# HITSZ-NRSL/De6D

Hardware: AMD Instinct MI355X
Metric: scenes/sec (16384-pt KITTI) at 1/2/4/8 MI355X; 3D mAP parity vs ref (higher is better)
Workload: dtype f32

## Files before the change

### de6d_amd/csrc/mlp_group.hip

```cpp
#include "common.h"
#include "compact_list.h"
#include "mfma_tile.h"

namespace {

D6_GEMM_PRIO_DECL


struct GroupArgs {
  int rows;
  const float *p; int ldp; int pcol0;
  const float *w1; int ldw1; const float *s1;
  const float *w2; int ldw2; const float *s2;
  const float *w3; int ldw3; const float *s3;
  const float *pts; int ldpts;
  const float *ctr; int ldctr;
  const int *idx; int n, m, ns; const int *cnt;
  const int *hdr; const int *crow_p; const int *crow_c;
  float *y; int ldy; int col0;
  int pre;
  int yvec;
  int *ticket;
};

__device__ __forceinline__ int g_draw_ticket(int *ticket, int grid) {
  return grid + __hip_atomic_fetch_add(ticket, 1, __ATOMIC_RELAXED, __HIP_MEMORY_SCOPE_AGENT);
}
__device__ __forceinline__ void g_leave(int *ticket, int workers) {
  const int gone = __hip_atomic_fetch_add(ticket + 1, 1, __ATOMIC_RELAXED, __HIP_MEMORY_SCOPE_AGENT);
  if (gone == workers - 1) {
    __hip_atomic_store(ticket, 0, __ATOMIC_RELAXED, __HIP_MEMORY_SCOPE_AGENT);
    __hip_atomic_store(ticket + 1, 0, __ATOMIC_RELAXED, __HIP_MEMORY_SCOPE_AGENT);
  }
}

template <int TN> constexpr int kGroupVW = TN >= 4 ? 4 : TN;
template <int TN>
__device__ __forceinline__ int tile_col(int j, int l31) {
  constexpr int VW = kGroupVW<TN>;
  return (j / VW) * (32 * VW) + VW * l31 + (j % VW);
}

template <int VW> struct BVec;
template <> struct BVec<1> { typedef float T; };
template <> struct BVec<2> { typedef f32x2 T; };
template <> struct BVec<4> { typedef f32x4 T; };

template <int VW>
__device__ __forceinline__ void g_store_group(float *rowptr, const float (&v)[VW], const int tag, float *__restrict__ scr,
                                              const int lane, const int yvec) {
  const bool live = tag >= 0;
  const int l31 = lane & 31;
  if constexpr (VW == 1) {
    if (live) d6_compact_store(rowptr + l31, v[0], tag);
  } else {
    if (!yvec) {
#pragma unroll
      for (int t = 0; t < VW; ++t)
        if (live) d6_compact_store(rowptr + VW * l31 + t, v[t], tag);
      return;
    }
    const bool atomic = live && (tag & kCompactTagSplit);
    typename BVec<VW>::T pack;
#pragma unroll
    for (int t = 0; t < VW; ++t) pack[t] = v[t];
    if (live && !atomic) *reinterpret_cast<typename BVec<VW>::T *>(rowptr + VW * l31) = pack;
    if (__ballot(atomic) != 0ull) {
      *reinterpret_cast<typename BVec<VW>::T *>(scr + lane * VW) = pack;
      d6_lds_wave_sync();
      const float *half = scr + (lane & 32) * VW;
      float x[VW];
#pragma unroll
      for (int t = 0; t < VW; ++t) x[t] = half[32 * t + l31];
      d6_lds_wave_sync();
      if (atomic) {
#pragma unroll
        for (int t = 0; t < VW; ++t)
          __hip_atomic_fetch_max(reinterpret_cast<int *>(rowptr + 32 * t + l31), __builtin_bit_cast(int, x[t]), __ATOMIC_RELAXED,
                                 __HIP_MEMORY_SCOPE_AGENT);
      }
    }
  }
}

template <int VW>
__device__ __forceinline__ typename BVec<VW>::T load_b(const __amdgpu_buffer_rsrc_t srd, uint32_t voff, int soff) {
  if constexpr (VW == 4) return __builtin_bit_cast(typename BVec<4>::T, __builtin_amdgcn_raw_buffer_load_b128(srd, voff, soff, 0));
  else if constexpr (VW == 2) return __builtin_bit_cast(typename BVec<2>::T, __builtin_amdgcn_raw_buffer_load_b64(srd, voff, soff, 0));
  else return __builtin_bit_cast(float, __builtin_amdgcn_raw_buffer_load_b32(srd, voff, soff, 0));
}
template <int VW>
__device__ __forceinline__ float bget(const typename BVec<VW>::T &v, int i) {
  if constexpr (VW == 1) return v;
  else return v[i];
}

#ifdef DET6D_EXPERIMENTS
__device__ int d6_group_kmul = 1;
#define D6_KOFF(x) (d6_group_kmul * (x))
__device__ int d6_group_phase_c2 = 512, d6_group_phase_c3 = 1024;
__device__ unsigned long long d6_group_phase[8 + 18];
#define D6_PHASE_DECL const unsigned long long ph_c0 = clock64(); unsigned long long ph_w3 = 0, ph_w2 = 0, ph_wt = 0; unsigned long long ph_t = wall_clock64(), ph_acc[5] = {0, 0, 0, 0, 0}, ph_tiles = 0; const unsigned long long ph_start = ph_t; const bool ph_on = C3 == d6_group_phase_c3 && C2 == d6_group_phase_c2;
#define D6_PHASE(i) do { if (ph_on) { __builtin_amdgcn_sched_barrier(0); const unsigned long long now_ = wall_clock64(); ph_acc[i] += now_ - ph_t; ph_t = now_; __builtin_amdgcn_sched_barrier(0); } } while (0)
#define D6_WAVE_T0 do { if (ph_on) { __builtin_amdgcn_sched_barrier(0); ph_wt = wall_clock64(); __builtin_amdgcn_sched_barrier(0); } } while (0)
#define D6_WAVE_T1(x) do { if (ph_on) { __builtin_amdgcn_sched_barrier(0); x += wall_clock64() - ph_wt; __builtin_amdgcn_sched_barrier(0); } } while (0)
#define D6_PHASE_END do { if (ph_on && tid == 0) { for (int i_ = 0; i_ < 5; ++i_) atomicAdd(&d6_group_phase[i_], ph_acc[i_]); atomicAdd(&d6_group_phase[5], ph_tiles); atomicAdd(&d6_group_phase[6], wall_clock64() - ph_start); atomicAdd(&d6_group_phase[7], 1ull); atomicAdd(&d6_group_phase[8], clock64() - ph_c0); } if (ph_on && (tid & 63) == 0) { atomicAdd(&d6_group_phase[9 + (tid >> 6)], ph_w3); atomicAdd(&d6_group_phase[17 + (tid >> 6)], ph_w2); } } while (0)
#else
#define D6_PHASE_DECL
#define D6_PHASE(i)
#define D6_WAVE_T0
#define D6_WAVE_T1(x)
#define D6_PHASE_END
#define D6_KOFF(x) (x)
#endif

template <int K, int TN, int LDX>
struct GroupLayer {
  static constexpr int VW = kGroupVW<TN>;
  static constexpr int NV = TN / VW;
  static constexpr int KS = K / 2;
  static constexpr int UK = 32 / TN;
  static constexpr int NB = KS / UK;
  static_assert(KS % UK == 0 && NB >= 2, "block structure");
  typedef typename BVec<VW>::T bvec;
  bvec b0[UK][NV], b1[UK][NV], b2[UK][NV];

  __device__ __forceinline__ static void fetch(bvec (&b)[UK][NV], const __amdgpu_buffer_rsrc_t srd, const uint32_t voff,
                                               const int ldw_bytes, const int blk) {
#pragma unroll
    for (int u = 0; u < UK; ++u)
#pragma unroll
      for (int v = 0; v < NV; ++v) b[u][v] = load_b<VW>(srd, voff, D6_KOFF(2 * (blk * UK + u) * ldw_bytes) + 128 * VW * v);
  }
  __device__ __forceinline__ static void compute(const bvec (&b)[UK][NV], const float *__restrict__ X, f32x16 (&acc)[TN],
                                                 const int l31, const int kh, const int blk) {
    float a[UK];
    const float *xa = X + l31 * LDX + 2 * blk * UK + kh;
#pragma unroll
    for (int u = 0; u < UK; ++u) a[u] = xa[2 * u];
#pragma unroll
    for (int u = 0; u < UK; ++u)
#pragma unroll
      for (int j = 0; j < TN; ++j) d6_mfma(a[u], bget<VW>(b[u][j / VW], j % VW), acc[j]);
  }
  __device__ __forceinline__ void start(const __amdgpu_buffer_rsrc_t srd, const uint32_t voff, const int ldw_bytes) {
    fetch(b0, srd, voff, ldw_bytes, 0);
    fetch(b1, srd, voff, ldw_bytes, 1);
  }
  __device__ __forceinline__ void run(const float *__restrict__ X, const __amdgpu_buffer_rsrc_t srd, const uint32_t voff,
                                      const int ldw_bytes, f32x16 (&acc)[TN], const int l31, const int kh) {
    auto clamp = [](int blk) { return blk < NB ? blk : NB - 1; };
    int blk = 0;
#pragma unroll 1
    for (; blk + 3 <= NB; blk += 3) {
      fetch(b2, srd, voff, ldw_bytes, blk + 2);
      compute(b0, X, acc, l31, kh, blk);
      fetch(b0, srd, voff, ldw_bytes, clamp(blk + 3));
      compute(b1, X, acc, l31, kh, blk + 1);
      fetch(b1, srd, voff, ldw_bytes, clamp(blk + 4));
      compute(b2, X, acc, l31, kh, blk + 2);
    }
    if (blk < NB) {
      compute(b0, X, acc, l31, kh, blk);
      if (blk + 1 < NB) compute(b1, X, acc, l31, kh, blk + 1);
    }
  }
};

template <bool COMPACT, int EPR>
__device__ __forceinline__ void group_row_entry(const GroupArgs &g, const int tile, const int tid, int &e0, int &e1) {
  const int r = tile * 32 + tid / EPR;
  if (COMPACT) { e0 = g.crow_c[r]; e1 = g.crow_p[r]; }
  else { e0 = g.idx[r]; e1 = 0; }
}

template <int C1, bool COMPACT, int EPR>
__device__ __forceinline__ void group_layer1(const GroupArgs &g, const int tile, const int tid, float *__restrict__ X1,
                                             int *__restrict__ tagbuf, const int e0, const int e1) {
  constexpr int LD1 = C1 + 1;
  const int erow = tid / EPR, eq = tid % EPR;
    {
      const int r = tile * 32 + erow;
      long long prow;
      int cj;
      bool real = true;
      if (COMPACT) {
        const int tag = e0;
        if (eq == 0) tagbuf[erow] = tag;
        real = tag >= 0;
        cj = d6_compact_centre(tag);
        prow = e1;
      } else {
        cj = r / g.ns;
        prow = (long long)(cj / g.m) * g.n + e0;
      }
      float dx = 0.f, dy = 0.f, dz = 0.f;
      if (real) {
        const float *pt = g.pts + prow * g.ldpts;
        const float *ce = g.ctr + (long long)cj * g.ldctr;
        dx = pt[0] - ce[0]; dy = pt[1] - ce[1]; dz = pt[2] - ce[2];
      }
      const float *prow_p = g.p + (real ? prow : 0) * g.ldp + g.pcol0;
      float *xr = X1 + erow * LD1;
#pragma unroll 4
      for (int c = 4 * eq; c < C1; c += 4 * EPR) {
        const f32x4 pv = *reinterpret_cast<const f32x4 *>(prow_p + c);
        const f32x4 wx = *reinterpret_cast<const f32x4 *>(g.w1 + c);
        const f32x4 wy = *reinterpret_cast<const f32x4 *>(g.w1 + g.ldw1 + c);
        const f32x4 wz = *reinterpret_cast<const f32x4 *>(g.w1 + 2 * g.ldw1 + c);
        const f32x4 sh = *reinterpret_cast<const f32x4 *>(g.s1 + c);
#pragma unroll
        for (int e = 0; e < 4; ++e) {
          const float v = d6_relu(D6_FMA(dz, wz[e], D6_FMA(dy, wy[e], D6_FMA(dx, wx[e], pv[e]))) + sh[e]);
          xr[c + e] = real ? v : 0.f;
        }
      }
    }
}

template <int TN3, bool COMPACT>
__device__ __forceinline__ void group_pool_store(const GroupArgs &g, const int tile, f32x16 (&acc)[TN3], const float (&sh3)[TN3],
                                                 const int colbase, const int l31, const int kh, const int h1, const int h2,
                                                 const int h3, const int h4, const int h5, const int *__restrict__ tagbuf,
                                                 float *__restrict__ scr) {
    constexpr int VW = kGroupVW<TN3>;
    constexpr int NG = TN3 / VW;
    const int lane = l31 + 32 * kh;
    if (COMPACT) {
      const int sc = d6_compact_class(tile * 32, h1, h2, h3, h4, h5);
      if (sc < 4) {
#pragma unroll
        for (int e = 0; e < 16; ++e) {
          if (sc == 2 && (e & 1)) continue;
          const int tag = tagbuf[d6_acc_row(e) + 4 * kh];
          float *dst = g.y + (size_t)(tag < 0 ? 0 : tag & kCompactTagCentre) * g.ldy + g.col0 + colbase;
#pragma unroll
          for (int jg = 0; jg < NG; ++jg) {
            float v[VW];
#pragma unroll
            for (int t = 0; t < VW; ++t) {
              const int j = jg * VW + t;
              const float raw = sc == 2 ? d6_vmax(acc[j][e], acc[j][e + 1 < 16 ? e + 1 : e]) : acc[j][e];
              v[t] = d6_compact_is_empty(tag) ? 0.f : d6_relu(raw + sh3[j]);
            }
            g_store_group<VW>(dst + jg * 32 * VW, v, tag, scr, lane, g.yvec);
          }
        }
      } else {
        int oc[4];
#pragma unroll
        for (int qq = 0; qq < 4; ++qq) {
          const int rr = d6_compact_out_row(sc, qq, kh);
          oc[qq] = rr >= 0 ? tagbuf[rr] : -1;
        }
#pragma unroll
        for (int jg = 0; jg < NG; ++jg) {
          float q[VW][4];
#pragma unroll
          for (int t = 0; t < VW; ++t) {
            const int j = jg * VW + t;
#pragma unroll
            for (int qq = 0; qq < 4; ++qq)
              q[t][qq] = d6_acc_max4(acc[j], qq);
            d6_compact_pool(q[t], sc);
          }
#pragma unroll
          for (int qq = 0; qq < 4; ++qq) {
            float v[VW];
#pragma unroll
            for (int t = 0; t < VW; ++t) v[t] = d6_compact_is_empty(oc[qq]) ? 0.f : d6_relu(q[t][qq] + sh3[jg * VW + t]);
            float *dst = g.y + (size_t)(oc[qq] < 0 ? 0 : oc[qq] & kCompactTagCentre) * g.ldy + g.col0 + colbase + jg * 32 * VW;
            g_store_group<VW>(dst, v, oc[qq], scr, lane, g.yvec);
          }
        }
      }
    } else {
      const int c0 = g.ns == 32 ? tile : 2 * tile;
      const int cnt0 = g.cnt[c0], cnt1 = g.ns == 32 ? 0 : g.cnt[c0 + 1];
      const int plain = kh == 0 ? 0 : -1;
#pragma unroll
      for (int jg = 0; jg < NG; ++jg) {
        float v0[VW], v1[VW];
#pragma unroll
        for (int t = 0; t < VW; ++t) {
          const int j = jg * VW + t;
          float q[4];
#pragma unroll
          for (int qq = 0; qq < 4; ++qq) q[qq] = d6_half_max(d6_acc_max4(acc[j], qq));
          if (g.ns == 32) {
            const float mx = d6_relu(d6_vmax(d6_vmax(q[0], q[1]), d6_vmax(q[2], q[3])) + sh3[j]);
            v0[t] = cnt0 > 0 ? mx : 0.f;
            v1[t] = 0.f;
          } else {
            v0[t] = cnt0 > 0 ? d6_relu(d6_vmax(q[0], q[1]) + sh3[j]) : 0.f;
            v1[t] = cnt1 > 0 ? d6_relu(d6_vmax(q[2], q[3]) + sh3[j]) : 0.f;
          }
        }
        float *dst = g.y + g.col0 + colbase + jg * 32 * VW;
        g_store_group<VW>(dst + (size_t)c0 * g.ldy, v0, plain, scr, lane, g.yvec);
        if (g.ns != 32) g_store_group<VW>(dst + (size_t)(c0 + 1) * g.ldy, v1, plain, scr, lane, g.yvec);
      }
    }
}

template <int C1, int C2, int C3, bool COMPACT, int NW>
__global__ __launch_bounds__(64 * NW, (NW == 4 && C3 <= 256) ? 3 : 1) void mlp_group_kernel(const GroupArgs g) {
  D6_GEMM_PRIO_APPLY();
  constexpr int LD1 = C1 + 1, LD2 = C2 + 1;
  constexpr int TN2 = C2 / (32 * NW), TN3 = C3 / (32 * NW);
  static_assert(TN2 >= 1 && TN3 >= 1, "every wave needs at least one 32-column tile per layer");
  extern __shared__ float lds[];
  float *X1 = lds;
  float *X2 = lds + 32 * LD1;
  int *tags = reinterpret_cast<int *>(lds + 32 * (LD1 + LD2));
  int it = 0;
  const int tid = threadIdx.x, lane = tid & 63, wave = tid >> 6, l31 = lane & 31, kh = lane >> 5;
  float *scr = reinterpret_cast<float *>(tags + 64) + wave * (64 * kGroupVW<TN3>);
  const int live_tiles = (COMPACT ? g.hdr[kCompactHdrLive] : g.rows) / 32;
  if ((int)blockIdx.x >= live_tiles) return;
  int h1 = 0, h2 = 0, h3 = 0, h4 = 0, h5 = 0;
  if (COMPACT) d6_compact_class_ends(g.hdr, h1, h2, h3, h4, h5);

  const __amdgpu_buffer_rsrc_t srd2 = d6_buffer(g.w2);
  const __amdgpu_buffer_rsrc_t srd3 = d6_buffer(g.w3);
  const uint32_t voff2 = (uint32_t)(kh * g.ldw2 + wave * (C2 / NW) + tile_col<TN2>(0, l31)) * 4u;
  const uint32_t voff3 = (uint32_t)(kh * g.ldw3 + wave * (C3 / NW) + tile_col<TN3>(0, l31)) * 4u;
  float sh2[TN2], sh3[TN3];
#pragma unroll
  for (int j = 0; j < TN2; ++j) sh2[j] = g.s2[wave * (C2 / NW) + tile_col<TN2>(j, l31)];
#pragma unroll
  for (int j = 0; j < TN3; ++j) sh3[j] = g.s3[wave * (C3 / NW) + tile_col<TN3>(j, l31)];

  D6_PHASE_DECL
  int e0, e1;
  group_row_entry<COMPACT, 2 * NW>(g, blockIdx.x, tid, e0, e1);
  __shared__ int next_tile_s[2];
  int *const ticket = COMPACT ? g.ticket : nullptr;
  for (int tile = blockIdx.x; tile < live_tiles;) {
#ifdef DET6D_EXPERIMENTS
    ++ph_tiles;
#endif
    int drawn = 0;
    if (ticket && tid == 0) drawn = g_draw_ticket(ticket, (int)gridDim.x);
    GroupLayer<C1, TN2, LD1> second;
    GroupLayer<C2, TN3, LD2> third;
    second.start(srd2, voff2, g.ldw2 * 4);
    const int par = it & 1;
    int *tagbuf = tags + 32 * (it++ & 1);
    if (!g.pre) group_row_entry<COMPACT, 2 * NW>(g, tile, tid, e0, e1);
    group_layer1<C1, COMPACT, 2 * NW>(g, tile, tid, X1, tagbuf, e0, e1);
    if (ticket && tid == 0) next_tile_s[par] = drawn;
    __syncthreads();
    const int next_tile = ticket ? next_tile_s[par] : tile + (int)gridDim.x;
    D6_PHASE(0);
    {
      f32x16 acc[TN2];
#pragma unroll
      for (int j = 0; j < TN2; ++j) d6_acc_zero(acc[j]);
      D6_WAVE_T0;
      second.run(X1, srd2, voff2, g.ldw2 * 4, acc, l31, kh);
      third.start(srd3, voff3, g.ldw3 * 4);
      D6_WAVE_T1(ph_w2);
      D6_PHASE(1);
#pragma unroll
      for (int j = 0; j < TN2; ++j) {
        float *xc = X2 + wave * (C2 / NW) + tile_col<TN2>(j, l31);
#pragma unroll
        for (int e = 0; e < 16; ++e) xc[(d6_acc_row(e) + 4 * kh) * LD2] = d6_relu(acc[j][e] + sh2[j]);
      }
    }
    __syncthreads();
    D6_PHASE(2);
    f32x16 acc[TN3];
#pragma unroll
    for (int j = 0; j < TN3; ++j) d6_acc_zero(acc[j]);
    D6_WAVE_T0;
    if (g.pre) {
      const int nt = next_tile;
      group_row_entry<COMPACT, 2 * NW>(g, nt < live_tiles ? nt : tile, tid, e0, e1);
    }
    third.run(X2, srd3, voff3, g.ldw3 * 4, acc, l31, kh);
    D6_WAVE_T1(ph_w3);
    D6_PHASE(3);
    group_pool_store<TN3, COMPACT>(g, tile, acc, sh3, wave * (C3 / NW), l31, kh, h1, h2, h3, h4, h5, tagbuf, scr);
    D6_PHASE(4);
    tile = next_tile;
  }
  if (ticket && tid == 0) g_leave(ticket, min((int)gridDim.x, live_tiles));
  D6_PHASE_END;
}


template <int K, int TN, int LDX, int UK, int DEPTH>
__device__ __forceinline__ void stream_layer(const float *__restrict__ X, const __amdgpu_buffer_rsrc_t srd, const uint32_t voff,
                                             const int ldw_bytes, const int soff0, f32x16 (&acc)[TN], const int l31, const int kh) {
  constexpr int VW = kGroupVW<TN>;
  constexpr int NV = TN / VW;
  constexpr int KS = K / 2;
  constexpr int NB = KS / UK;
  static_assert(KS % UK == 0 && NB % DEPTH == 0 && NB >= DEPTH, "ring structure");
  typedef typename BVec<VW>::T bvec;
  bvec b[DEPTH][UK][NV];
  auto fetch = [&](bvec (&bs)[UK][NV], int blk) {
#pragma unroll
    for (int u = 0; u < UK; ++u)
#pragma unroll
      for (int v = 0; v < NV; ++v) bs[u][v] = load_b<VW>(srd, voff, soff0 + D6_KOFF(2 * (blk * UK + u) * ldw_bytes) + 128 * VW * v);
  };
  const float *xa = X + l31 * LDX + kh;
  float a[UK];
#pragma unroll
  for (int d = 0; d < DEPTH - 1; ++d) fetch(b[d], d);
#pragma unroll
  for (int u = 0; u < UK; ++u) a[u] = xa[2 * u];
#pragma unroll 1
  for (int blk = 0; blk < NB; blk += DEPTH) {
#pragma unroll
    for (int d = 0; d < DEPTH; ++d) {
      const int cur = blk + d;
      fetch(b[(d + DEPTH - 1) % DEPTH], cur + DEPTH - 1 < NB ? cur + DEPTH - 1 : NB - 1);
      float an[UK];
      const int nxt = cur + 1 < NB ? cur + 1 : cur;
#pragma unroll
      for (int u = 0; u < UK; ++u) an[u] = xa[2 * (nxt * UK + u)];
#pragma unroll
      for (int u = 0; u < UK; ++u)
#pragma unroll
        for (int j = 0; j < TN; ++j) d6_mfma(a[u], bget<VW>(b[d][u][j / VW], j % VW), acc[j]);
#pragma unroll
      for (int u = 0; u < UK; ++u) a[u] = an[u];
    }
  }
}

template <int C1, int C2, int C3, bool COMPACT>
__global__ __launch_bounds__(256, 2) void mlp_group_stream_kernel(const GroupArgs g) {
  D6_GEMM_PRIO_APPLY();
  constexpr int CH = 128;
  constexpr int NCH = C2 / CH;
  constexpr int LD1 = C1 + 1, LDY = CH + 1;
  constexpr int TN3 = C3 / 128;
  static_assert(C2 % CH == 0 && NCH >= 2 && TN3 >= 2, "chunk structure");
  extern __shared__ float lds[];
  float *X1 = lds;
  float *Y0 = lds + 32 * LD1;
  float *Y1 = Y0 + 32 * LDY;
  int *tags = reinterpret_cast<int *>(Y1 + 32 * LDY);
  int it = 0;
  const int tid = threadIdx.x, lane = tid & 63, wave = tid >> 6, l31 = lane & 31, kh = lane >> 5;
  float *scr = reinterpret_cast<float *>(tags + 64) + wave * (64 * kGroupVW<TN3>);
  const int live_tiles = (COMPACT ? g.hdr[kCompactHdrLive] : g.rows) / 32;
  if ((int)blockIdx.x >= live_tiles) return;
  int h1 = 0, h2 = 0, h3 = 0, h4 = 0, h5 = 0;
  if (COMPACT) d6_compact_class_ends(g.hdr, h1, h2, h3, h4, h5);

  const __amdgpu_buffer_rsrc_t srd2 = d6_buffer(g.w2);
  const __amdgpu_buffer_rsrc_t srd3 = d6_buffer(g.w3);
  const uint32_t voff2 = (uint32_t)(kh * g.ldw2 + 32 * wave + l31) * 4u;
  const uint32_t voff3 = (uint32_t)(kh * g.ldw3 + wave * (C3 / 4) + tile_col<TN3>(0, l31)) * 4u;
  float sh3[TN3];
#pragma unroll
  for (int j = 0; j < TN3; ++j) sh3[j] = g.s3[wave * (C3 / 4) + tile_col<TN3>(j, l31)];

  auto second = [&](const int c, float *__restrict__ Y) {
    const float sh2 = g.s2[CH * c + 32 * wave + l31];
    f32x16 acc2[1];
    d6_acc_zero(acc2[0]);
    stream_layer<C1, 1, LD1, 8, 4>(X1, srd2, voff2, g.ldw2 * 4, CH * c * 4, acc2, l31, kh);
    float *yc = Y + 32 * wave + l31;
#pragma unroll
    for (int e = 0; e < 16; ++e) yc[(d6_acc_row(e) + 4 * kh) * LDY] = d6_relu(acc2[0][e] + sh2);
  };

  __shared__ int next_tile_s[2];
  int *const ticket = COMPACT ? g.ticket : nullptr;
  for (int tile = blockIdx.x; tile < live_tiles;) {
    int drawn = 0;
    if (ticket && tid == 0) drawn = g_draw_ticket(ticket, (int)gridDim.x);
    const int par = it & 1;
    int *tagbuf = tags + 32 * (it++ & 1);
    int e0, e1;
    group_row_entry<COMPACT, 8>(g, tile, tid, e0, e1);
    group_layer1<C1, COMPACT, 8>(g, tile, tid, X1, tagbuf, e0, e1);
    if (ticket && tid == 0) next_tile_s[par] = drawn;
    __syncthreads();
    const int next_tile = ticket ? next_tile_s[par] : tile + (int)gridDim.x;
    f32x16 acc[TN3];
#pragma unroll
    for (int j = 0; j < TN3; ++j) d6_acc_zero(acc[j]);
    second(0, Y0);
    __syncthreads();
#pragma unroll 1
    for (int c = 0; c < NCH; ++c) {
      float *Yc = (c & 1) ? Y1 : Y0;
      float *Yn = (c & 1) ? Y0 : Y1;
      stream_layer<CH, TN3, LDY, 16 / TN3 >= 1 ? 16 / TN3 : 1, 4>(Yc, srd3, voff3, g.ldw3 * 4, CH * c * g.ldw3 * 4, acc, l31, kh);
      if (c + 1 < NCH) {
        second(c + 1, Yn);
        __syncthreads();
      }
    }
    group_pool_store<TN3, COMPACT>(g, tile, acc, sh3, wave * (C3 / 4), l31, kh, h1, h2, h3, h4, h5, tagbuf, scr);
    tile = next_tile;
  }
  if (ticket && tid == 0) g_leave(ticket, min((int)gridDim.x, live_tiles));
}

static int group_grid(int rows, size_t lds_bytes, int max_per_cu) {
  int per_cu = (int)((160 * 1024) / lds_bytes);
  per_cu = per_cu < 1 ? 1 : (per_cu > max_per_cu ? max_per_cu : per_cu);
  const int blocks = rows / 32;
  return blocks > 256 * per_cu ? 256 * per_cu : blocks;
}

template <int C1, int C2, int C3, bool COMPACT>
int launch_group_stream(const GroupArgs &g, hipStream_t stream) {
  const size_t lds_bytes = sizeof(float) * (32 * (size_t)(C1 + 1 + 2 * 129) + 64 + 4 * 64 * kGroupVW<C3 / 128>);
  DET6D_MAX_DYNAMIC_LDS((mlp_group_stream_kernel<C1, C2, C3, COMPACT>), lds_bytes);
  const int blocks = group_grid(g.rows, lds_bytes, 3);
  hipLaunchKernelGGL((mlp_group_stream_kernel<C1, C2, C3, COMPACT>), dim3(blocks), dim3(256), lds_bytes, stream, g);
  return det6d_check_launch("det6d_mlp_group3 (streaming)");
}

template <int C1, int C2, int C3, bool COMPACT, int NW>
int launch_group(const GroupArgs &g, hipStream_t stream) {
  const size_t lds_bytes = sizeof(float) * (32 * (size_t)(C1 + 1 + C2 + 1) + 64 + NW * 64 * kGroupVW<C3 / (32 * NW)>);
  DET6D_MAX_DYNAMIC_LDS((mlp_group_kernel<C1, C2, C3, COMPACT, NW>), lds_bytes);
  const int blocks = group_grid(g.rows, lds_bytes, 4);
#ifdef DET6D_EXPERIMENTS
  static bool phase_set = false;
  if (!phase_set) {
    const int pc2 = det6d_env_int("DET6D_GROUP_PHASE_C2", 512), pc3 = det6d_env_int("DET6D_GROUP_PHASE_C3", 1024);
    hipMemcpyToSymbol(HIP_SYMBOL(d6_group_phase_c2), &pc2, sizeof(int));
    hipMemcpyToSymbol(HIP_SYMBOL(d6_group_phase_c3), &pc3, sizeof(int));
    phase_set = true;
  }
  static const int whatif = det6d_env_int("DET6D_GROUP_WHATIF", 0);
  static bool whatif_set = false;
  if (whatif && !whatif_set) {
    const int zero = 0;
    hipMemcpyToSymbol(HIP_SYMBOL(d6_group_kmul), &zero, sizeof(int));
    whatif_set = true;
  }
#endif
  hipLaunchKernelGGL((mlp_group_kernel<C1, C2, C3, COMPACT, NW>), dim3(blocks), dim3(64 * NW), lds_bytes, stream, g);
  return det6d_check_launch("det6d_mlp_group3");
}

}

#ifdef DET6D_EXPERIMENTS
extern "C" __attribute__((visibility("default"))) int det6d_dbg_group_phase(unsigned long long *out_host) {
  if (hipMemcpyFromSymbol(out_host, HIP_SYMBOL(d6_group_phase), sizeof(unsigned long long) * 26) != hipSuccess) return -1;
  const unsigned long long zero[26] = {0};
  return hipMemcpyToSymbol(HIP_SYMBOL(d6_group_phase), zero, sizeof(zero)) == hipSuccess ? 0 : -1;
}
#endif

static bool group_widths_ok(int c1, int c2, int c3) {
  return (c1 == 128 && c2 == 128 && c3 == 256) || (c1 == 128 && c2 == 256 && c3 == 256) || (c1 == 256 && c2 == 256 && c3 == 512) ||
         (c1 == 256 && c2 == 512 && c3 == 1024);
}

DET6D_API int det6d_mlp_group3_supported(int c1, int c2, int c3, int ns, int compact) {
  return group_widths_ok(c1, c2, c3) && (compact || ns == 16 || ns == 32) ? 1 : 0;
}

DET6D_API int det6d_mlp_group3(int rows, const float *p, int ldp, int pcol0, const float *w1, int ldw1, const float *s1, int c1,
                               const float *w2, int ldw2, const float *s2, int c2, const float *w3, int ldw3, const float *s3,
                               int c3, const float *pts, int ldpts, const float *ctr, int ldctr, const int *idx, int n, int m,
                               int ns, const int *cnt, int *hdr, const int *crow_p, const int *crow_c, float *y, int ldy,
                               int col0, det6d_stream_t stream) {
  D6_GEMM_PRIO_HOST();
  if (rows < 0 || (rows & 31) || !p || !w1 || !w2 || !w3 || !s1 || !s2 || !s3 || !pts || !ctr || !y) return DET6D_EINVAL;
  if (!group_widths_ok(c1, c2, c3)) return DET6D_EINVAL;
  if ((ldp & 3) || (pcol0 & 3) || (ldw1 & 3) || ldp < pcol0 + c1 || ldw1 < c1 || ldw2 < c2 || ldw3 < c3 || ldpts < 3 || ldctr < 3)
    return DET6D_EINVAL;
  if (((uintptr_t)p | (uintptr_t)w1 | (uintptr_t)s1) & 15) return DET6D_EINVAL;
  if ((size_t)c1 * ldw2 * 4 >= 0xfff00000ull || (size_t)c2 * ldw3 * 4 >= 0xfff00000ull) return DET6D_EINVAL;
  const bool compact = hdr != nullptr;
  if (compact ? (!crow_p || !crow_c || (rows & 127)) : (!idx || !cnt || n <= 0 || m <= 0 || (ns != 16 && ns != 32) || rows % (m * ns)))
    return DET6D_EINVAL;
  if (!compact && ns == 16 && (m & 1)) return DET6D_EINVAL;
  if (rows == 0) return DET6D_OK;
  GroupArgs g;
  g.rows = rows; g.p = p; g.ldp = ldp; g.pcol0 = pcol0;
  g.w1 = w1; g.ldw1 = ldw1; g.s1 = s1; g.w2 = w2; g.ldw2 = ldw2; g.s2 = s2; g.w3 = w3; g.ldw3 = ldw3; g.s3 = s3;
  g.pts = pts; g.ldpts = ldpts; g.ctr = ctr; g.ldctr = ldctr;
  g.idx = idx; g.n = n; g.m = m; g.ns = ns; g.cnt = cnt;
  g.hdr = hdr; g.crow_p = crow_p; g.crow_c = crow_c;
  static const int static_tiles = det6d_env_int("DET6D_GROUP_STATIC", 0);
  g.ticket = (hdr && !static_tiles) ? hdr + kCompactHdrTicket : nullptr;
  g.y = y; g.ldy = ldy; g.col0 = col0;
  static const int pre_entries = det6d_env_int("DET6D_GROUP_PRE", 1);
  g.pre = pre_entries;
  g.yvec = (!(ldy & 3) && !(col0 & 3) && !((uintptr_t)y & 15)) ? 1 : 0;
  hipStream_t s = (hipStream_t)stream;
  static const int nw_env = det6d_env_int("DET6D_GROUP_WAVES", 0);
  static const int stream_form = det6d_env_int("DET6D_GROUP_STREAM", 3);
  if ((stream_form & 1) && c1 == 256 && c2 == 512 && c3 == 1024)
    return compact ? launch_group_stream<256, 512, 1024, true>(g, s) : launch_group_stream<256, 512, 1024, false>(g, s);
  if ((stream_form & 2) && c1 == 256 && c2 == 256 && c3 == 512)
    return compact ? launch_group_stream<256, 256, 512, true>(g, s) : launch_group_stream<256, 256, 512, false>(g, s);
  if ((stream_form & 4) && c1 == 128 && c2 == 256 && c3 == 256)
    return compact ? launch_group_stream<128, 256, 256, true>(g, s) : launch_group_stream<128, 256, 256, false>(g, s);
#define D6_GROUP(A, B, C, NWD)                                                                        \
  if (c1 == A && c2 == B && c3 == C) {                                                                \
    if ((nw_env ? nw_env : NWD) == 8 && B >= 256)                                                     \
      return compact ? launch_group<A, B, C, true, (B >= 256 ? 8 : 4)>(g, s) : launch_group<A, B, C, false, (B >= 256 ? 8 : 4)>(g, s); \
    return compact ? launch_group<A, B, C, true, 4>(g, s) : launch_group<A, B, C, false, 4>(g, s);    \
  }
  static const int sa3_waves = det6d_env_int("DET6D_GROUP_SA3_WAVES", 4);
  D6_GROUP(128, 128, 256, 4)
  if (sa3_waves != 8) { D6_GROUP(128, 256, 256, 4) }
  D6_GROUP(128, 256, 256, 8)
  D6_GROUP(256, 256, 512, 8)
  D6_GROUP(256, 512, 1024, 8)
#undef D6_GROUP
  return DET6D_EINVAL;
}
```

Before: 12790.

## Software-pipeline layer-1 weight loads and stage W1 in LDS for streaming kernel

Restructures the first grouped-MLP layer so all point features are issued up front and the weight rows are prefetched a few iterations ahead, with sched barriers to keep the loads hoisted. The ticket draw moves inside so its atomic latency overlaps those loads. For the streaming kernel with wide inputs, W1 and the shift are staged once per block in LDS, and row indices for the next tile are prefetched when pre-computation is on. The shared next-tile slot now lives in dynamic LDS. This costs extra registers and LDS, which may reduce occupancy.

```diff
diff --git a/de6d_amd/csrc/mlp_group.hip b/de6d_amd/csrc/mlp_group.hip
--- a/de6d_amd/csrc/mlp_group.hip
+++ b/de6d_amd/csrc/mlp_group.hip
@@ -174,48 +174,75 @@
   else { e0 = g.idx[r]; e1 = 0; }
 }
 
-template <int C1, bool COMPACT, int EPR>
+template <int C1>
+__device__ __forceinline__ void group_stage_w1(const GroupArgs &g, const int tid, const int nthreads, float *__restrict__ W1s) {
+  for (int c = 4 * tid; c < 4 * C1; c += 4 * nthreads) {
+    const int row = c / C1, col = c % C1;
+    const float *src = row < 3 ? g.w1 + row * g.ldw1 + col : g.s1 + col;
+    *reinterpret_cast<f32x4 *>(W1s + c) = *reinterpret_cast<const f32x4 *>(src);
+  }
+}
+
+template <int C1, bool COMPACT, int EPR, bool W1S, int WB>
 __device__ __forceinline__ void group_layer1(const GroupArgs &g, const int tile, const int tid, float *__restrict__ X1,
-                                             int *__restrict__ tagbuf, const int e0, const int e1) {
+                                             int *__restrict__ tagbuf, const int e0, const int e1, const float *__restrict__ W1s,
+                                             int *const ticket, int &drawn) {
   constexpr int LD1 = C1 + 1;
+  constexpr int NI = C1 / (4 * EPR);
+  static_assert(C1 % (4 * EPR) == 0 && NI >= 1, "a row's columns divide evenly among its EPR threads");
   const int erow = tid / EPR, eq = tid % EPR;
-    {
-      const int r = tile * 32 + erow;
-      long long prow;
-      int cj;
-      bool real = true;
-      if (COMPACT) {
-        const int tag = e0;
-        if (eq == 0) tagbuf[erow] = tag;
-        real = tag >= 0;
-        cj = d6_compact_centre(tag);
-        prow = e1;
-      } else {
-        cj = r / g.ns;
-        prow = (long long)(cj / g.m) * g.n + e0;
-      }
-      float dx = 0.f, dy = 0.f, dz = 0.f;
-      if (real) {
-        const float *pt = g.pts + prow * g.ldpts;
-        const float *ce = g.ctr + (long long)cj * g.ldctr;
-        dx = pt[0] - ce[0]; dy = pt[1] - ce[1]; dz = pt[2] - ce[2];
-      }
-      const float *prow_p = g.p + (real ? prow : 0) * g.ldp + g.pcol0;
-      float *xr = X1 + erow * LD1;
-#pragma unroll 4
-      for (int c = 4 * eq; c < C1; c += 4 * EPR) {
-        const f32x4 pv = *reinterpret_cast<const f32x4 *>(prow_p + c);
-        const f32x4 wx = *reinterpret_cast<const f32x4 *>(g.w1 + c);
-        const f32x4 wy = *reinterpret_cast<const f32x4 *>(g.w1 + g.ldw1 + c);
-        const f32x4 wz = *reinterpret_cast<const f32x4 *>(g.w1 + 2 * g.ldw1 + c);
-        const f32x4 sh = *reinterpret_cast<const f32x4 *>(g.s1 + c);
-#pragma unroll
-        for (int e = 0; e < 4; ++e) {
-          const float v = d6_relu(D6_FMA(dz, wz[e], D6_FMA(dy, wy[e], D6_FMA(dx, wx[e], pv[e]))) + sh[e]);
-          xr[c + e] = real ? v : 0.f;
-        }
-      }
-    }
+  const int r = tile * 32 + erow;
+  long long prow;
+  int cj;
+  bool real = true;
+  if (COMPACT) {
+    const int tag = e0;
+    if (eq == 0) tagbuf[erow] = tag;
+    real = tag >= 0;
+    cj = real ? d6_compact_centre(tag) : 0;
+    prow = real ? e1 : 0;
+  } else {
+    cj = r / g.ns;
+    prow = (long long)(cj / g.m) * g.n + e0;
+  }
+  const float *prow_p = g.p + prow * g.ldp + g.pcol0 + 4 * eq;
+  const float *pt = g.pts + prow * g.ldpts;
+  const float *ce = g.ctr + (long long)cj * g.ldctr;
+  f32x4 pv[NI], wx[NI], wy[NI], wz[NI], sh[NI];
+  const float *wrow = (W1S ? W1s : g.w1) + 4 * eq, *srow = (W1S ? W1s + 3 * C1 : g.s1) + 4 * eq;
+  const int ldw = W1S ? C1 : g.ldw1;
+  auto fetch_w = [&](const int i) {
+    wx[i] = *reinterpret_cast<const f32x4 *>(wrow + 4 * EPR * i);
+    wy[i] = *reinterpret_cast<const f32x4 *>(wrow + ldw + 4 * EPR * i);
+    wz[i] = *reinterpret_cast<const f32x4 *>(wrow + 2 * ldw + 4 * EPR * i);
+    sh[i] = *reinterpret_cast<const f32x4 *>(srow + 4 * EPR * i);
+  };
+#pragma unroll
+  for (int i = 0; i < NI; ++i) pv[i] = *reinterpret_cast<const f32x4 *>(prow_p + 4 * EPR * i);
+  float px = pt[0], py = pt[1], pz = pt[2];
+  const float cx = ce[0], cy = ce[1], cz = ce[2];
+#pragma unroll
+  for (int i = 0; i < (WB < NI ? WB : NI); ++i) fetch_w(i);
+  __builtin_amdgcn_sched_barrier(0);
+  if (ticket && tid == 0) drawn = g_draw_ticket(ticket, (int)gridDim.x);
+  float *xr = X1 + erow * LD1 + 4 * eq;
+  float dx = 0.f, dy = 0.f, dz = 0.f;
+#pragma unroll
+  for (int i = 0; i < NI; ++i) {
+    if (i + WB < NI) {
+      fetch_w(i + WB);
+      __builtin_amdgcn_sched_barrier(0);
+    }
+    if (i == 0) {
+      asm volatile("" : "+v"(px), "+v"(py), "+v"(pz));
+      dx = px - cx; dy = py - cy; dz = pz - cz;
+    }
+#pragma unroll
+    for (int e = 0; e < 4; ++e) {
+      const float v = d6_relu(D6_FMA(dz, wz[i][e], D6_FMA(dy, wy[i][e], D6_FMA(dx, wx[i][e], pv[i][e]))) + sh[i][e]);
+      xr[4 * EPR * i + e] = real ? v : 0.f;
+    }
+  }
 }
 
 template <int TN3, bool COMPACT>
@@ -307,6 +334,7 @@
 __global__ __launch_bounds__(64 * NW, (NW == 4 && C3 <= 256) ? 3 : 1) void mlp_group_kernel(const GroupArgs g) {
   D6_GEMM_PRIO_APPLY();
   constexpr int LD1 = C1 + 1, LD2 = C2 + 1;
+  constexpr int WB1 = NW == 4 ? (C3 <= 256 ? 1 : 2) : 4;
   constexpr int TN2 = C2 / (32 * NW), TN3 = C3 / (32 * NW);
   static_assert(TN2 >= 1 && TN3 >= 1, "every wave needs at least one 32-column tile per layer");
   extern __shared__ float lds[];
@@ -316,6 +344,7 @@
   int it = 0;
   const int tid = threadIdx.x, lane = tid & 63, wave = tid >> 6, l31 = lane & 31, kh = lane >> 5;
   float *scr = reinterpret_cast<float *>(tags + 64) + wave * (64 * kGroupVW<TN3>);
+  int *next_tile_s = reinterpret_cast<int *>(reinterpret_cast<float *>(tags + 64) + NW * (64 * kGroupVW<TN3>));
   const int live_tiles = (COMPACT ? g.hdr[kCompactHdrLive] : g.rows) / 32;
   if ((int)blockIdx.x >= live_tiles) return;
   int h1 = 0, h2 = 0, h3 = 0, h4 = 0, h5 = 0;
@@ -334,21 +363,19 @@
   D6_PHASE_DECL
   int e0, e1;
   group_row_entry<COMPACT, 2 * NW>(g, blockIdx.x, tid, e0, e1);
-  __shared__ int next_tile_s[2];
   int *const ticket = COMPACT ? g.ticket : nullptr;
   for (int tile = blockIdx.x; tile < live_tiles;) {
 #ifdef DET6D_EXPERIMENTS
     ++ph_tiles;
 #endif
     int drawn = 0;
-    if (ticket && tid == 0) drawn = g_draw_ticket(ticket, (int)gridDim.x);
     GroupLayer<C1, TN2, LD1> second;
     GroupLayer<C2, TN3, LD2> third;
     second.start(srd2, voff2, g.ldw2 * 4);
     const int par = it & 1;
     int *tagbuf = tags + 32 * (it++ & 1);
     if (!g.pre) group_row_entry<COMPACT, 2 * NW>(g, tile, tid, e0, e1);
-    group_layer1<C1, COMPACT, 2 * NW>(g, tile, tid, X1, tagbuf, e0, e1);
+    group_layer1<C1, COMPACT, 2 * NW, false, WB1>(g, tile, tid, X1, tagbuf, e0, e1, nullptr, ticket, drawn);
     if (ticket && tid == 0) next_tile_s[par] = drawn;
     __syncthreads();
     const int next_tile = ticket ? next_tile_s[par] : tile + (int)gridDim.x;
@@ -433,6 +460,8 @@
   }
 }
 
+template <int C1> constexpr bool kStreamStagesW1 = C1 >= 256;
+
 template <int C1, int C2, int C3, bool COMPACT>
 __global__ __launch_bounds__(256, 2) void mlp_group_stream_kernel(const GroupArgs g) {
   D6_GEMM_PRIO_APPLY();
@@ -441,6 +470,7 @@
   constexpr int LD1 = C1 + 1, LDY = CH + 1;
   constexpr int TN3 = C3 / 128;
   static_assert(C2 % CH == 0 && NCH >= 2 && TN3 >= 2, "chunk structure");
+  constexpr bool W1S = kStreamStagesW1<C1>;
   extern __shared__ float lds[];
   float *X1 = lds;
   float *Y0 = lds + 32 * LD1;
@@ -449,6 +479,8 @@
   int it = 0;
   const int tid = threadIdx.x, lane = tid & 63, wave = tid >> 6, l31 = lane & 31, kh = lane >> 5;
   float *scr = reinterpret_cast<float *>(tags + 64) + wave * (64 * kGroupVW<TN3>);
+  float *W1s = reinterpret_cast<float *>(tags + 64) + 4 * (64 * kGroupVW<TN3>);
+  int *next_tile_s = reinterpret_cast<int *>(W1s + (W1S ? 4 * C1 : 0));
   const int live_tiles = (COMPACT ? g.hdr[kCompactHdrLive] : g.rows) / 32;
   if ((int)blockIdx.x >= live_tiles) return;
   int h1 = 0, h2 = 0, h3 = 0, h4 = 0, h5 = 0;
@@ -472,19 +504,26 @@
     for (int e = 0; e < 16; ++e) yc[(d6_acc_row(e) + 4 * kh) * LDY] = d6_relu(acc2[0][e] + sh2);
   };
 
-  __shared__ int next_tile_s[2];
+  int e0, e1;
+  group_row_entry<COMPACT, 8>(g, blockIdx.x, tid, e0, e1);
+  if (W1S) {
+    group_stage_w1<C1>(g, tid, 256, W1s);
+    __syncthreads();
+  }
   int *const ticket = COMPACT ? g.ticket : nullptr;
   for (int tile = blockIdx.x; tile < live_tiles;) {
     int drawn = 0;
-    if (ticket && tid == 0) drawn = g_draw_ticket(ticket, (int)gridDim.x);
     const int par = it & 1;
     int *tagbuf = tags + 32 * (it++ & 1);
-    int e0, e1;
-    group_row_entry<COMPACT, 8>(g, tile, tid, e0, e1);
-    group_layer1<C1, COMPACT, 8>(g, tile, tid, X1, tagbuf, e0, e1);
+    if (!g.pre) group_row_entry<COMPACT, 8>(g, tile, tid, e0, e1);
+    group_layer1<C1, COMPACT, 8, W1S, 4>(g, tile, tid, X1, tagbuf, e0, e1, W1s, ticket, drawn);
     if (ticket && tid == 0) next_tile_s[par] = drawn;
     __syncthreads();
     const int next_tile = ticket ? next_tile_s[par] : tile + (int)gridDim.x;
+    if (g.pre) {
+      const int nt = next_tile;
+      group_row_entry<COMPACT, 8>(g, nt < live_tiles ? nt : tile, tid, e0, e1);
+    }
     f32x16 acc[TN3];
 #pragma unroll
     for (int j = 0; j < TN3; ++j) d6_acc_zero(acc[j]);
@@ -515,7 +554,8 @@
 
 template <int C1, int C2, int C3, bool COMPACT>
 int launch_group_stream(const GroupArgs &g, hipStream_t stream) {
-  const size_t lds_bytes = sizeof(float) * (32 * (size_t)(C1 + 1 + 2 * 129) + 64 + 4 * 64 * kGroupVW<C3 / 128>);
+  const size_t lds_bytes = sizeof(float) * (32 * (size_t)(C1 + 1 + 2 * 129) + 64 + 4 * 64 * kGroupVW<C3 / 128> +
+                                            (kStreamStagesW1<C1> ? 4 * C1 : 0) + 4);
   DET6D_MAX_DYNAMIC_LDS((mlp_group_stream_kernel<C1, C2, C3, COMPACT>), lds_bytes);
   const int blocks = group_grid(g.rows, lds_bytes, 3);
   hipLaunchKernelGGL((mlp_group_stream_kernel<C1, C2, C3, COMPACT>), dim3(blocks), dim3(256), lds_bytes, stream, g);
@@ -524,7 +564,7 @@
 
 template <int C1, int C2, int C3, bool COMPACT, int NW>
 int launch_group(const GroupArgs &g, hipStream_t stream) {
-  const size_t lds_bytes = sizeof(float) * (32 * (size_t)(C1 + 1 + C2 + 1) + 64 + NW * 64 * kGroupVW<C3 / (32 * NW)>);
+  const size_t lds_bytes = sizeof(float) * (32 * (size_t)(C1 + 1 + C2 + 1) + 64 + NW * 64 * kGroupVW<C3 / (32 * NW)> + 4);
   DET6D_MAX_DYNAMIC_LDS((mlp_group_kernel<C1, C2, C3, COMPACT, NW>), lds_bytes);
   const int blocks = group_grid(g.rows, lds_bytes, 4);
 #ifdef DET6D_EXPERIMENTS
```

New measurement: 13000, median of 6. 1.02x the previous value.
